# lucasnewman/f5-tts-mlx

Hardware: NVIDIA H100
Metric: mel-frames/sec (higher is better)
Workload: dtype bf16

## Files before the change

### f5_tts_mlx_b200/csrc/gemm_epilogue.cuh

```cuda
#pragma once
#include "ptx.cuh"

namespace f5 {

enum GemmAct { ACT_NONE = 0, ACT_GELU_TANH = 1, ACT_GELU_ERF = 2, ACT_MISH = 3 };

struct GemmParams {
  int M, N, K;
  int rows_per_batch;
  int tiles_per_batch;
  int num_batches;
  int conv_taps;
  int conv_pad;
  int k_per_tap;
  int conv_grouped;
  const float* bias;
  void* out;
  int ldo;
  const float* resid;
  int ldr;
  const float* gate;
  const int* row_len;
  const float2* rope;
  int rope_cols;
  int rope_col2;
  float q_scale;
  int q_cols;
  __nv_bfloat16* out2;
  int ldo2;
  unsigned long long* prof;
  int w_static;
  const char* pf_ptr;
  long long pf_bytes;
  const float* ln_scale;
  float2* ln_stats;
  const float2* ln_in_stats;
  int ln_in_units;
  const float* ln_tab;
  long long ln_tab_ld;
  int ab8;
  float acc_scale;
  int out2_fp8;
  int out_fp8;
  const float* a_scale;
  long long a_scale_ld;
  const float* w_scale;
  float* out_scale;
  float* out2_scale;
  int conv_dilation;
};

__device__ __forceinline__ void prefetch_slice_l2(const GemmParams& p, int cta, int num_ctas, int lane) {
  if (p.pf_ptr == nullptr) return;
  const long long per = (((p.pf_bytes + num_ctas - 1) / num_ctas) + 127) & ~127LL;
  const long long lo = (long long)cta * per;
  const long long hi = lo + per < p.pf_bytes ? lo + per : p.pf_bytes;
  for (long long o = lo + (long long)lane * 128; o < hi; o += 32 * 128)
    asm volatile("prefetch.global.L2 [%0];" ::"l"(p.pf_ptr + o));
}

__device__ __forceinline__ float tanh_approx(float x) {
  float y;
  asm("tanh.approx.f32 %0, %1;" : "=f"(y) : "f"(x));
  return y;
}
__device__ __forceinline__ float gelu_tanh_fast(float x) {
  const float k0 = 0.7978845608028654f, k1 = 0.044715f;
  const float u = k0 * fmaf(k1 * x * x, x, x);
  return 0.5f * x * (1.f + tanh_approx(u));
}
__device__ __forceinline__ float mish_fast(float x) {
  const float sp = x > 15.f ? x : __logf(1.f + __expf(x));
  return x * tanh_approx(sp);
}

template <int BN, bool SC = false>
__device__ __forceinline__ void epi_stage_cols(const GemmParams& p, int n0, int et, float* bias_s,
                                               float* gate_s, float* aux_s, float* ws_s = nullptr) {
#pragma unroll
  for (int i = et; i < BN; i += 128) {
    const int col = n0 + i;
    const bool ok = col < p.N;
    if constexpr (SC) ws_s[i] = (p.w_scale != nullptr && ok) ? p.acc_scale * p.w_scale[col] : p.acc_scale;
    float b = (p.bias != nullptr && ok) ? p.bias[col] : 0.f;
    float x = (p.ln_scale != nullptr && ok) ? 1.f + p.ln_scale[col] : 1.f;
    if (p.ln_in_stats != nullptr && ok) {
      const float* t = p.ln_tab + col;
      x = t[0] + t[p.ln_tab_ld];
      b += t[2 * p.ln_tab_ld] + t[3 * p.ln_tab_ld];
    }
    bias_s[i] = b;
    gate_s[i] = (p.gate != nullptr && ok) ? p.gate[col] : 1.f;
    aux_s[i] = x;
  }
}

__device__ __forceinline__ void epi_load_ln_row(const GemmParams& p, int row, bool row_ok, float& mu_r, float& rstd) {
  mu_r = 0.f; rstd = 1.f;
  if (p.ln_in_stats == nullptr || !row_ok) return;
  const float4* st = reinterpret_cast<const float4*>(p.ln_in_stats + (size_t)row * p.ln_in_units);
  float s1 = 0.f, s2 = 0.f;
  for (int u = 0; u < p.ln_in_units; u += 2) {
    const float4 v = st[u >> 1];
    s1 += v.x; s2 += v.y;
    s1 += v.z; s2 += v.w;
  }
  const float inv_k = 1.f / (64.f * p.ln_in_units);
  const float mean = s1 * inv_k;
  rstd = rsqrtf(fmaxf(s2 * inv_k - mean * mean, 0.f) + 1e-6f);
  mu_r = mean * rstd;
}

template <bool ROPE>
__device__ __forceinline__ void epi_load_rope(const GemmParams& p, int pos, float2 (&cs)[ROPE ? 32 : 1]) {
  if (ROPE) {
    const float4* rp = reinterpret_cast<const float4*>(p.rope + (size_t)pos * 32);
#pragma unroll
    for (int j = 0; j < 16; ++j) {
      const float4 v = rp[j];
      cs[2 * j] = make_float2(v.x, v.y);
      cs[2 * j + 1] = make_float2(v.z, v.w);
    }
  }
}

__device__ __forceinline__ void epi_load_resid(const GemmParams& p, int row, int col0, bool row_ok,
                                               float4 (&r)[8]) {
  if (p.resid != nullptr && row_ok && col0 < p.N) {
    const float4* rr = reinterpret_cast<const float4*>(p.resid + (size_t)row * p.ldr + col0);
#pragma unroll
    for (int j = 0; j < 8; ++j) r[j] = (col0 + 4 * j < p.N) ? rr[j] : make_float4(0.f, 0.f, 0.f, 0.f);
  } else {
#pragma unroll
    for (int j = 0; j < 8; ++j) r[j] = make_float4(0.f, 0.f, 0.f, 0.f);
  }
}

struct EpiStage {
  uint8_t* acc;
  uint8_t* stg;
  int et;
  int r;
  int bar_id;
  const CUtensorMap* map_out;
  const CUtensorMap* map_out2;
  int c1, c2;
  int out_fp8;
  float mu_r, rstd;
};

__device__ __forceinline__ void epi_stage_f32(uint8_t* buf, int r, const float (&v)[32]) {
  uint8_t* mine = buf + r * 128;
  const int sw = r & 7;
#pragma unroll
  for (int j = 0; j < 8; ++j)
    *reinterpret_cast<float4*>(mine + ((j ^ sw) * 16)) = make_float4(v[4 * j], v[4 * j + 1], v[4 * j + 2], v[4 * j + 3]);
}

template <bool OUT_BF16>
__device__ __forceinline__ void epi_store_tma(const float (&v)[32], const EpiStage& st, int ch, int col0,
                                              const uint4* w2 = nullptr, bool w2_fp8 = false) {
  uint8_t* box = st.acc + ch * 16384;
  uint8_t* buf = st.stg + (ch & 1) * 8192;
  if (OUT_BF16 && st.out_fp8) {
    uint8_t* mine = buf + st.r * 32;
    const int sw = (st.r >> 2) & 1;
#pragma unroll
    for (int j = 0; j < 2; ++j)
      *reinterpret_cast<uint4*>(mine + ((j ^ sw) * 16)) =
          make_uint4(pack_e4m3x4(v[16 * j], v[16 * j + 1], v[16 * j + 2], v[16 * j + 3]),
                     pack_e4m3x4(v[16 * j + 4], v[16 * j + 5], v[16 * j + 6], v[16 * j + 7]),
                     pack_e4m3x4(v[16 * j + 8], v[16 * j + 9], v[16 * j + 10], v[16 * j + 11]),
                     pack_e4m3x4(v[16 * j + 12], v[16 * j + 13], v[16 * j + 14], v[16 * j + 15]));
  } else if (OUT_BF16) {
    uint8_t* mine = buf + st.r * 64;
    const int sw = (st.r >> 1) & 3;
#pragma unroll
    for (int j = 0; j < 4; ++j)
      *reinterpret_cast<uint4*>(mine + ((j ^ sw) * 16)) =
          make_uint4(pack_bf16x2(v[8 * j], v[8 * j + 1]), pack_bf16x2(v[8 * j + 2], v[8 * j + 3]),
                     pack_bf16x2(v[8 * j + 4], v[8 * j + 5]), pack_bf16x2(v[8 * j + 6], v[8 * j + 7]));
  } else {
    epi_stage_f32(box, st.r, v);
  }
  if (w2 != nullptr) {
    if (w2_fp8) {
      uint8_t* mine2 = buf + st.r * 32;
      const int sw2 = (st.r >> 2) & 1;
#pragma unroll
      for (int j = 0; j < 2; ++j) *reinterpret_cast<uint4*>(mine2 + ((j ^ sw2) * 16)) = w2[j];
    } else {
      uint8_t* mine2 = buf + st.r * 64;
      const int sw2 = (st.r >> 1) & 3;
#pragma unroll
      for (int j = 0; j < 4; ++j) *reinterpret_cast<uint4*>(mine2 + ((j ^ sw2) * 16)) = w2[j];
    }
  }
  fence_proxy_async_smem();
  if (st.et == 0) tma_store_wait_read<0>();
  asm volatile("bar.sync %0, 128;" ::"r"(st.bar_id) : "memory");
  if (st.et == 0) {
    tma_store_3d(st.map_out, OUT_BF16 ? buf : box, col0, st.c1, st.c2);
    if (w2 != nullptr) tma_store_3d(st.map_out2, buf, col0, st.c1, st.c2);
    tma_store_commit();
  }
}


__device__ __forceinline__ void epi_quant32(const float (&v)[32], const float* aux, float inv, uint4 (&q)[2]) {
  uint32_t w[8];
#pragma unroll
  for (int i = 0; i < 8; ++i) {
    float x[4];
#pragma unroll
    for (int k = 0; k < 4; ++k) x[k] = (aux != nullptr ? v[4 * i + k] * aux[4 * i + k] : v[4 * i + k]) * inv;
    w[i] = pack_e4m3x4(x[0], x[1], x[2], x[3]);
  }
  q[0] = make_uint4(w[0], w[1], w[2], w[3]);
  q[1] = make_uint4(w[4], w[5], w[6], w[7]);
}

__device__ __forceinline__ void epi_quant32_staged(const uint8_t* buf, int r, const float* aux, float inv, uint4 (&q)[2]) {
  const uint8_t* mine = buf + r * 128;
  const int sw = r & 7;
  uint32_t w[8];
#pragma unroll
  for (int i = 0; i < 8; ++i) {
    const float4 a = *reinterpret_cast<const float4*>(mine + ((i ^ sw) * 16));
    float x[4] = {a.x, a.y, a.z, a.w};
#pragma unroll
    for (int k = 0; k < 4; ++k) x[k] = (aux != nullptr ? x[k] * aux[4 * i + k] : x[k]) * inv;
    w[i] = pack_e4m3x4(x[0], x[1], x[2], x[3]);
  }
  q[0] = make_uint4(w[0], w[1], w[2], w[3]);
  q[1] = make_uint4(w[4], w[5], w[6], w[7]);
}

template <bool OUT_BF16>
__device__ __forceinline__ void epi_finish_unit8(const float (&v)[32], const float* aux, float amax, float* scale,
                                                 int M, int colA, int row, bool row_ok, const EpiStage& st, int chA) {
  float inv;
  const float s = e4m3_block_scale(amax, inv);
  if (row_ok) scale[(size_t)(colA >> 6) * M + row] = s;
  uint8_t* q8 = st.stg + ((chA >> 1) & 1) * 8192;
  const int sw = (st.r >> 2) & 1;
  {
    uint4 q[2];
    epi_quant32(v, aux, inv, q);
#pragma unroll
    for (int j = 0; j < 2; ++j) *reinterpret_cast<uint4*>(q8 + 4096 + st.r * 32 + ((j ^ sw) * 16)) = q[j];
  }
  uint8_t* box_b = st.acc + (chA + 1) * 16384;
  if constexpr (!OUT_BF16) epi_stage_f32(box_b, st.r, v);
  {
    uint4 q[2];
    epi_quant32_staged(st.acc + chA * 16384, st.r, aux != nullptr ? aux - 32 : nullptr, inv, q);
#pragma unroll
    for (int j = 0; j < 2; ++j) *reinterpret_cast<uint4*>(q8 + st.r * 32 + ((j ^ sw) * 16)) = q[j];
  }
  fence_proxy_async_smem();
  if (st.et == 0) tma_store_wait_read<0>();
  asm volatile("bar.sync %0, 128;" ::"r"(st.bar_id) : "memory");
  if (st.et == 0) {
    if constexpr (!OUT_BF16) tma_store_3d(st.map_out, box_b, colA + 32, st.c1, st.c2);
    const CUtensorMap* m8 = OUT_BF16 ? st.map_out : st.map_out2;
    tma_store_3d(m8, q8, colA, st.c1, st.c2);
    tma_store_3d(m8, q8 + 4096, colA + 32, st.c1, st.c2);
    tma_store_commit();
  }
}

template <int ACT, bool OUT_BF16, bool ROPE, int HALF, bool SC = false>
__device__ __forceinline__ void epi_apply(const uint32_t (&acc)[32], const float4 (&res)[8],
                                          const float* bias_s, const float* gate_s, const float* aux_s,
                                          const float2 (&cs)[ROPE ? 32 : 1], const GemmParams& p,
                                          int col0, int ch, int row, bool row_ok, bool row_valid,
                                          const EpiStage& st, float2& unit_acc, const float* ws_s = nullptr,
                                          float* unit_amax = nullptr) {
  float v[32];
  if constexpr (SC) {
#pragma unroll
    for (int j = 0; j < 32; j += 4) {
      const float4 bb = *reinterpret_cast<const float4*>(bias_s + j);
      const float4 cc = *reinterpret_cast<const float4*>(aux_s + j);
      const float4 ww = *reinterpret_cast<const float4*>(ws_s + j);
      v[j] = fmaf(__uint_as_float(acc[j]), st.rstd * ww.x, fmaf(-st.mu_r, cc.x, bb.x));
      v[j + 1] = fmaf(__uint_as_float(acc[j + 1]), st.rstd * ww.y, fmaf(-st.mu_r, cc.y, bb.y));
      v[j + 2] = fmaf(__uint_as_float(acc[j + 2]), st.rstd * ww.z, fmaf(-st.mu_r, cc.z, bb.z));
      v[j + 3] = fmaf(__uint_as_float(acc[j + 3]), st.rstd * ww.w, fmaf(-st.mu_r, cc.w, bb.w));
    }
  } else if (p.ln_in_stats != nullptr) {
    const float ra = st.rstd * p.acc_scale;
#pragma unroll
    for (int j = 0; j < 32; j += 4) {
      const float4 bb = *reinterpret_cast<const float4*>(bias_s + j);
      const float4 cc = *reinterpret_cast<const float4*>(aux_s + j);
      v[j] = fmaf(__uint_as_float(acc[j]), ra, fmaf(-st.mu_r, cc.x, bb.x));
      v[j + 1] = fmaf(__uint_as_float(acc[j + 1]), ra, fmaf(-st.mu_r, cc.y, bb.y));
      v[j + 2] = fmaf(__uint_as_float(acc[j + 2]), ra, fmaf(-st.mu_r, cc.z, bb.z));
      v[j + 3] = fmaf(__uint_as_float(acc[j + 3]), ra, fmaf(-st.mu_r, cc.w, bb.w));
    }
  } else {
#pragma unroll
    for (int j = 0; j < 32; j += 4) {
      const float4 bb = *reinterpret_cast<const float4*>(bias_s + j);
      v[j] = fmaf(__uint_as_float(acc[j]), p.acc_scale, bb.x);
      v[j + 1] = fmaf(__uint_as_float(acc[j + 1]), p.acc_scale, bb.y);
      v[j + 2] = fmaf(__uint_as_float(acc[j + 2]), p.acc_scale, bb.z);
      v[j + 3] = fmaf(__uint_as_float(acc[j + 3]), p.acc_scale, bb.w);
    }
  }
  if (ACT == ACT_GELU_TANH) {
#pragma unroll
    for (int j = 0; j < 32; ++j) v[j] = gelu_tanh_fast(v[j]);
  } else if (ACT == ACT_GELU_ERF) {
#pragma unroll
    for (int j = 0; j < 32; ++j) v[j] = gelu_erf_f(v[j]);
  } else if (ACT == ACT_MISH) {
#pragma unroll
    for (int j = 0; j < 32; ++j) v[j] = mish_fast(v[j]);
  }
  if (ROPE) {
    if (col0 < p.rope_cols || (unsigned)(col0 - p.rope_col2) < (unsigned)p.rope_cols) {
#pragma unroll
      for (int j = 0; j < 16; ++j) {
        const float2 c = cs[HALF * 16 + j];
        const float a = v[2 * j], b = v[2 * j + 1];
        v[2 * j] = a * c.x - b * c.y;
        v[2 * j + 1] = b * c.x + a * c.y;
      }
    }
    if (col0 < p.q_cols) {
#pragma unroll
      for (int j = 0; j < 32; ++j) v[j] *= p.q_scale;
    }
  }
  if (p.row_len != nullptr) {
    if (!row_valid) {
#pragma unroll
      for (int j = 0; j < 32; ++j) v[j] = 0.f;
    }
  }
#pragma unroll
  for (int j = 0; j < 8; ++j) {
    const float4 gg = *reinterpret_cast<const float4*>(gate_s + 4 * j);
    v[4 * j] = fmaf(v[4 * j], gg.x, res[j].x); v[4 * j + 1] = fmaf(v[4 * j + 1], gg.y, res[j].y);
    v[4 * j + 2] = fmaf(v[4 * j + 2], gg.z, res[j].z); v[4 * j + 3] = fmaf(v[4 * j + 3], gg.w, res[j].w);
  }
  if constexpr (!OUT_BF16) {
    if (p.out2 != nullptr) {
      if (p.ln_stats != nullptr) {
        float s1[4] = {HALF == 0 ? 0.f : unit_acc.x, 0.f, 0.f, 0.f}, s2[4] = {HALF == 0 ? 0.f : unit_acc.y, 0.f, 0.f, 0.f};
#pragma unroll
        for (int j = 0; j < 32; j += 4) {
#pragma unroll
          for (int i = 0; i < 4; ++i) { s1[i] += v[j + i]; s2[i] = fmaf(v[j + i], v[j + i], s2[i]); }
        }
        unit_acc = make_float2((s1[0] + s1[1]) + (s1[2] + s1[3]), (s2[0] + s2[1]) + (s2[2] + s2[3]));
        if (HALF == 1 && row_ok && col0 < p.N) p.ln_stats[(size_t)row * (p.N >> 6) + (col0 >> 6)] = unit_acc;
      }
      if constexpr (SC) {
        if (p.out2_fp8 && p.out2_scale != nullptr) {
          float amax = HALF == 0 ? 0.f : *unit_amax;
#pragma unroll
          for (int j = 0; j < 32; ++j) amax = fmax_nan(amax, fabsf(v[j] * aux_s[j]));
          if (HALF == 0) {
            *unit_amax = amax;
            epi_store_tma<OUT_BF16>(v, st, ch, col0);
          } else {
            epi_finish_unit8<OUT_BF16>(v, aux_s, amax, p.out2_scale, p.M, col0 - 32, row, row_ok, st, ch - 1);
          }
          return;
        }
      }
      uint4 w2[4];
      if (p.out2_fp8) {
#pragma unroll
        for (int j = 0; j < 2; ++j) {
          uint32_t q[4];
#pragma unroll
          for (int i = 0; i < 4; ++i) {
            const float4 sc = *reinterpret_cast<const float4*>(aux_s + 16 * j + 4 * i);
            q[i] = pack_e4m3x4(v[16 * j + 4 * i] * sc.x, v[16 * j + 4 * i + 1] * sc.y, v[16 * j + 4 * i + 2] * sc.z,
                               v[16 * j + 4 * i + 3] * sc.w);
          }
          w2[j] = make_uint4(q[0], q[1], q[2], q[3]);
        }
      } else {
#pragma unroll
        for (int j = 0; j < 4; ++j) {
          const float4 s0 = *reinterpret_cast<const float4*>(aux_s + 8 * j);
          const float4 s1 = *reinterpret_cast<const float4*>(aux_s + 8 * j + 4);
          w2[j] = make_uint4(pack_bf16x2(v[8 * j] * s0.x, v[8 * j + 1] * s0.y), pack_bf16x2(v[8 * j + 2] * s0.z, v[8 * j + 3] * s0.w),
                             pack_bf16x2(v[8 * j + 4] * s1.x, v[8 * j + 5] * s1.y), pack_bf16x2(v[8 * j + 6] * s1.z, v[8 * j + 7] * s1.w));
        }
      }
      epi_store_tma<OUT_BF16>(v, st, ch, col0, w2, p.out2_fp8 != 0);
      return;
    }
  }
  if constexpr (SC && OUT_BF16) {
    if (st.out_fp8 && p.out_scale != nullptr) {
      float amax = HALF == 0 ? 0.f : *unit_amax;
#pragma unroll
      for (int j = 0; j < 32; ++j) amax = fmax_nan(amax, fabsf(v[j]));
      if (HALF == 0) {
        *unit_amax = amax;
        epi_stage_f32(st.acc + ch * 16384, st.r, v);
      } else {
        epi_finish_unit8<OUT_BF16>(v, nullptr, amax, p.out_scale, p.M, col0 - 32, row, row_ok, st, ch - 1);
      }
      return;
    }
  }
  epi_store_tma<OUT_BF16>(v, st, ch, col0);
}

__device__ __forceinline__ void acc_ld32(const uint8_t* box, int r, uint32_t (&acc)[32]) {
  const uint8_t* mine = box + r * 128;
  const int sw = r & 7;
#pragma unroll
  for (int j = 0; j < 8; ++j) {
    const float4 v = *reinterpret_cast<const float4*>(mine + ((j ^ sw) * 16));
    acc[4 * j] = __float_as_uint(v.x); acc[4 * j + 1] = __float_as_uint(v.y);
    acc[4 * j + 2] = __float_as_uint(v.z); acc[4 * j + 3] = __float_as_uint(v.w);
  }
}

template <int BN, int ACT, bool OUT_BF16, bool ROPE, bool SC = false>
__device__ __forceinline__ void epi_drain_tile(const float* bias_s, const float* gate_s, const float* aux_s,
                                               const float2 (&cs)[ROPE ? 32 : 1], float4 (&res0)[8], const GemmParams& p,
                                               int n0, int row, bool row_ok, bool row_valid, const EpiStage& st,
                                               const float* ws_s = nullptr) {
  float4 res1[8];
  float2 unit_acc = make_float2(0.f, 0.f);
  float unit_amax = 0.f;
#pragma unroll 1
  for (int cc = 0; cc < BN / 64; ++cc) {
    const int colA = n0 + cc * 64, colB = colA + 32;
    uint32_t acc[32];
    constexpr bool kLateB = ROPE || SC;
    if (kLateB || cc > 0) epi_load_resid(p, row, colA, row_ok, res0);
    if constexpr (!kLateB) epi_load_resid(p, row, colB, row_ok, res1);
    acc_ld32(st.acc + (2 * cc) * 16384, st.r, acc);
    if (colA < p.N)
      epi_apply<ACT, OUT_BF16, ROPE, 0, SC>(acc, res0, bias_s + cc * 64, gate_s + cc * 64, aux_s + cc * 64, cs, p, colA,
                                            2 * cc, row, row_ok, row_valid, st, unit_acc, SC ? ws_s + cc * 64 : nullptr,
                                            &unit_amax);
    if constexpr (kLateB) epi_load_resid(p, row, colB, row_ok, res1);
    acc_ld32(st.acc + (2 * cc + 1) * 16384, st.r, acc);
    if (colB < p.N)
      epi_apply<ACT, OUT_BF16, ROPE, 1, SC>(acc, res1, bias_s + cc * 64 + 32, gate_s + cc * 64 + 32, aux_s + cc * 64 + 32, cs,
                                            p, colB, 2 * cc + 1, row, row_ok, row_valid, st, unit_acc,
                                            SC ? ws_s + cc * 64 + 32 : nullptr, &unit_amax);
  }
}

}
```

### f5_tts_mlx_b200/csrc/gemm_sm90.cuh

```cuda
#pragma once
#include <type_traits>

#include "ptx.cuh"
#include "gemm_epilogue.cuh"

namespace f5 {

template <int BN, int kStages, bool SCALED = false>
struct GemmSmem {
  static constexpr int kABytes = 128 * 128;
  static constexpr int kBBytes = BN * 128;
  static constexpr int kStageBytes = kABytes + kBBytes;
  static constexpr int kAccOffset = kStages * kStageBytes;
  static constexpr int kAccBytes = (BN / 32) * 16384;
  static constexpr int kStgOffset = kAccOffset + kAccBytes;
  static constexpr int kBarOffset = kStgOffset + 16384;
  static constexpr int kColsOffset = (kBarOffset + (2 * kStages + 2) * 8 + 15) & ~15;
  static constexpr int kTotal = kColsOffset + (SCALED ? 4 : 3) * BN * 4 + 1024;
  static_assert(kStageBytes % 1024 == 0, "SWIZZLE_128B tiles and boxes sit on 1024-byte boundaries");
  static_assert(kTotal <= 232448, "GEMM: shared memory over the 227 KB limit");
};

template <int BN>
struct GemmEpi {
  static constexpr int kThreads = 384;
};

template <int BN, bool AB8>
__device__ __forceinline__ void gemm_wgmma(float (&acc)[BN / 2], uint64_t da, uint64_t db, uint32_t scale_d) {
  if constexpr (AB8) {
    if constexpr (BN == 128) wgmma_e4m3_ss_n128(acc, da, db, scale_d);
    else wgmma_e4m3_ss_n64(acc, da, db, scale_d);
  } else {
    if constexpr (BN == 128) wgmma_bf16_ss_n128(acc, da, db, scale_d);
    else wgmma_bf16_ss_n64(acc, da, db, scale_d);
  }
}

struct GemmTile {
  int n0;
  int batch;
  int m_in_batch0;
  int row0;
};
__device__ __forceinline__ GemmTile gemm_tile(const GemmParams& p, int t, int bn) {
  GemmTile g;
  const int tiles_n = (p.N + bn - 1) / bn;
  const int mt = t / tiles_n;
  g.n0 = (t - mt * tiles_n) * bn;
  if (p.tiles_per_batch > 0) {
    g.batch = mt / p.tiles_per_batch;
    g.m_in_batch0 = (mt - g.batch * p.tiles_per_batch) * 128;
    g.row0 = g.batch * p.rows_per_batch + g.m_in_batch0;
  } else {
    g.batch = 0;
    g.row0 = mt * 128;
    g.m_in_batch0 = g.row0;
  }
  return g;
}
__device__ __forceinline__ int gemm_tiles(const GemmParams& p, int bn) {
  return (p.N + bn - 1) / bn * (p.tiles_per_batch > 0 ? p.num_batches * p.tiles_per_batch : (p.M + 127) / 128);
}
__device__ __forceinline__ int gemm_num_kb(const GemmParams& p) {
  return p.conv_taps * (p.ab8 ? (p.k_per_tap + 127) >> 7 : (p.k_per_tap + 63) >> 6);
}

template <int BN, int kStages, int ACT, bool OUT_BF16, bool ROPE, bool FP8 = false, bool RESID = true, bool SCALED = false>
__global__ void __launch_bounds__(384, 1)
gemm_bf16_tn_kernel(const __grid_constant__ CUtensorMap tma_a,
                    const __grid_constant__ CUtensorMap tma_b, const __grid_constant__ CUtensorMap tma_out,
                    const __grid_constant__ CUtensorMap tma_out2, const GemmParams p_arg) {
  GemmParams p = p_arg;
  if constexpr (!FP8) { p.ab8 = 0; p.out_fp8 = 0; p.out2_fp8 = 0; p.acc_scale = 1.f; }
  if constexpr (!RESID) p.resid = nullptr;
  if constexpr (!SCALED) { p.a_scale = nullptr; p.w_scale = nullptr; p.out_scale = nullptr; p.out2_scale = nullptr; }
  using S = GemmSmem<BN, kStages, SCALED>;
  extern __shared__ uint8_t smem_raw[];
  uint8_t* smem = smem_raw + ((1024u - (smem_u32(smem_raw) & 1023u)) & 1023u);
  uint64_t* full_bar = reinterpret_cast<uint64_t*>(smem + S::kBarOffset);
  uint64_t* empty_bar = full_bar + kStages;
  uint64_t* mma_turn = empty_bar + kStages;
  uint64_t* epi_free = mma_turn + 1;

  const int warp = threadIdx.x >> 5;
  const int lane = threadIdx.x & 31;

  if (warp == 0 && elect_one()) {
    tma_prefetch_desc(&tma_a);
    tma_prefetch_desc(&tma_b);
    tma_prefetch_desc(&tma_out);
    if (p.out2 != nullptr) tma_prefetch_desc(&tma_out2);
    for (int i = 0; i < kStages; ++i) {
      mbar_init(&full_bar[i], 1);
      mbar_init(&empty_bar[i], 128);
    }
    mbar_init(mma_turn, 128);
    mbar_init(epi_free, 128);
    fence_mbar_init();
  }
  if (warp == 1) prefetch_slice_l2(p, blockIdx.x, gridDim.x, lane);
  __syncthreads();
  const int early_b = p.w_static ? min(kStages, gemm_num_kb(p)) : 0;
  if (warp == 0 && elect_one()) {
    const int n0 = gemm_tile(p, blockIdx.x, BN).n0;
    for (int kb = 0; kb < early_b; ++kb) {
      mbar_expect_tx(&full_bar[kb], S::kStageBytes);
      tma_load_2d(smem + kb * S::kStageBytes + S::kABytes, &tma_b, &full_bar[kb], kb * (p.ab8 ? 128 : 64), n0);
    }
  }
  pdl_wait();
  if (threadIdx.x == 128) prof_stamp_begin(p.prof);

  if (warp < 4) {
    asm volatile("setmaxnreg.dec.sync.aligned.u32 40;\n");
    if (warp == 0 && elect_one()) {
      auto produce = [&](auto ab8_tag) {
        constexpr int KBE = decltype(ab8_tag)::value ? 128 : 64;
        const int kb_per_tap = (p.k_per_tap + KBE - 1) / KBE, num_kb = p.conv_taps * kb_per_tap, tiles = gemm_tiles(p, BN);
        const int tap_step = p.conv_dilation > 1 ? p.conv_dilation : 1;
        int s = 0;
        uint32_t ph = 1;
        uint8_t* sa = smem;
        int early = p.w_static ? min(kStages, num_kb) : 0;
        for (int t = blockIdx.x; t < tiles; t += gridDim.x) {
          const GemmTile g = gemm_tile(p, t, BN);
          const int a_col0 = p.conv_grouped ? g.n0 : 0;
          int a_row = g.m_in_batch0 - p.conv_pad, kc = 0;
          for (int kb = 0; kb < num_kb; ++kb) {
            mbar_wait(&empty_bar[s], ph);
            if (kb >= early) mbar_expect_tx(&full_bar[s], S::kStageBytes);
            tma_load_3d(sa, &tma_a, &full_bar[s], a_col0 + kc * KBE, a_row, g.batch);
            if (kb >= early) tma_load_2d(sa + S::kABytes, &tma_b, &full_bar[s], kb * KBE, g.n0);
            if (++s == kStages) { s = 0; ph ^= 1; sa = smem; } else { sa += S::kStageBytes; }
            if (++kc == kb_per_tap) { kc = 0; a_row += tap_step; }
          }
          early = 0;
        }
      };
      if (p.ab8) produce(std::true_type{});
      else produce(std::false_type{});
    }
  } else {
    asm volatile("setmaxnreg.inc.sync.aligned.u32 232;\n");
    const int wg = (threadIdx.x >> 7) - 1;
    const int et = threadIdx.x & 127;
    const int wr = ((threadIdx.x >> 5) & 3) * 16 + (lane >> 2);
    const uint32_t ring = smem_u32(smem);
    uint8_t* acc_tile = smem + S::kAccOffset;
    float* bias_s = reinterpret_cast<float*>(smem + S::kColsOffset);
    float* gate_s = bias_s + BN;
    float* aux_s = bias_s + 2 * BN;
    float* ws_s = SCALED ? bias_s + 3 * BN : nullptr;

    const uint32_t turn_par = (uint32_t)wg ^ 1u;
#pragma unroll 1
    for (int t = blockIdx.x + wg * gridDim.x; t < gemm_tiles(p, BN); t += 2 * gridDim.x) {
      const int num_kb = gemm_num_kb(p);
      const bool first = t == (int)blockIdx.x;
      const int kb0 = (t - (int)blockIdx.x) / (int)gridDim.x * num_kb;
      int s = kb0 % kStages;
      uint32_t ph = (uint32_t)(kb0 / kStages) & 1u;
      if (!first) mbar_wait(mma_turn, turn_par);

      float acc[2][BN / 2];
#pragma unroll
      for (int h = 0; h < 2; ++h)
#pragma unroll
        for (int i = 0; i < BN / 2; ++i) acc[h][i] = 0.f;
      auto mma_loop = [&](auto ab8_tag) {
        constexpr bool AB8 = decltype(ab8_tag)::value;
        if constexpr (AB8) {
          float part[BN / 2];
          for (int kb = 0; kb < num_kb; ++kb) {
            mbar_wait(&full_bar[s], ph);
            const uint32_t sa = ring + s * S::kStageBytes, sb = ring + s * S::kStageBytes + S::kABytes;
#pragma unroll
            for (int h = 0; h < 2; ++h) {
              wgmma_fence();
#pragma unroll
              for (int k = 0; k < 4; ++k)
                gemm_wgmma<BN, true>(part, gmma_desc_sw128(sa + h * (64 * 128) + 32 * k, 16, 1024),
                                     gmma_desc_sw128(sb + 32 * k, 16, 1024), k != 0);
              wgmma_commit();
              wgmma_wait<0>();
              wgmma_reg_fence(part);
              if (h == 1) mbar_arrive(&empty_bar[s]);
#pragma unroll
              for (int i = 0; i < BN / 2; ++i) acc[h][i] += part[i];
            }
            if (++s == kStages) { s = 0; ph ^= 1; }
          }
        } else {
          int s_prev = 0;
          for (int kb = 0; kb < num_kb; ++kb) {
            mbar_wait(&full_bar[s], ph);
            const uint32_t sa = ring + s * S::kStageBytes, sb = ring + s * S::kStageBytes + S::kABytes;
            wgmma_fence();
#pragma unroll
            for (int h = 0; h < 2; ++h)
#pragma unroll
              for (int k = 0; k < 4; ++k)
                gemm_wgmma<BN, false>(acc[h], gmma_desc_sw128(sa + h * (64 * 128) + 32 * k, 16, 1024),
                                      gmma_desc_sw128(sb + 32 * k, 16, 1024), (kb | k) != 0);
            wgmma_commit();
            wgmma_wait<1>();
            if (kb > 0) mbar_arrive(&empty_bar[s_prev]);
            s_prev = s;
            if (++s == kStages) { s = 0; ph ^= 1; }
          }
          wgmma_wait<0>();
          wgmma_reg_fence(acc[0]);
          wgmma_reg_fence(acc[1]);
          mbar_arrive(&empty_bar[s_prev]);
        }
      };
      auto mma_loop_scaled = [&]() {
        const GemmTile g = gemm_tile(p, t, BN);
        const int lim = p.tiles_per_batch > 0 ? p.rows_per_batch - g.m_in_batch0 : p.M - g.row0;
        const float* sp = p.a_scale + g.row0 + wr;
        const size_t ld = (size_t)p.a_scale_ld;
        float part[BN / 2];
        for (int kb = 0; kb < num_kb; ++kb) {
          float sc[2][2][2];
#pragma unroll
          for (int u = 0; u < 2; ++u) {
            const float* su = sp + (size_t)(2 * kb + u) * ld;
#pragma unroll
            for (int h = 0; h < 2; ++h) {
              sc[u][h][0] = 64 * h + wr < lim ? su[64 * h] : 0.f;
              sc[u][h][1] = 64 * h + wr + 8 < lim ? su[64 * h + 8] : 0.f;
            }
          }
          mbar_wait(&full_bar[s], ph);
          const uint32_t sa = ring + s * S::kStageBytes, sb = ring + s * S::kStageBytes + S::kABytes;
#pragma unroll
          for (int u = 0; u < 2; ++u) {
#pragma unroll
            for (int h = 0; h < 2; ++h) {
              wgmma_fence();
#pragma unroll
              for (int k = 0; k < 2; ++k)
                gemm_wgmma<BN, true>(part, gmma_desc_sw128(sa + h * (64 * 128) + 64 * u + 32 * k, 16, 1024),
                                     gmma_desc_sw128(sb + 64 * u + 32 * k, 16, 1024), k != 0);
              wgmma_commit();
              wgmma_wait<0>();
              wgmma_reg_fence(part);
              if (u == 1 && h == 1) mbar_arrive(&empty_bar[s]);
#pragma unroll
              for (int i = 0; i < BN / 2; ++i) acc[h][i] = fmaf(part[i], sc[u][h][(i >> 1) & 1], acc[h][i]);
            }
          }
          if (++s == kStages) { s = 0; ph ^= 1; }
        }
      };
      if constexpr (SCALED) {
        if (p.ab8 && p.a_scale != nullptr) mma_loop_scaled();
        else if (p.ab8) mma_loop(std::true_type{});
        else mma_loop(std::false_type{});
      } else {
        if (p.ab8) mma_loop(std::true_type{});
        else mma_loop(std::false_type{});
      }
      mbar_arrive(mma_turn);
      if (t + (int)gridDim.x >= gemm_tiles(p, BN)) pdl_launch_dependents();

      const GemmTile g = gemm_tile(p, t, BN);
      if (!first) mbar_wait(epi_free, turn_par);
      {
        const int sw = wr & 7;
        uint8_t* base = acc_tile + wr * 128 + (lane & 1) * 8;
#pragma unroll
        for (int h = 0; h < 2; ++h)
#pragma unroll
          for (int q = 0; q < BN / 8; ++q) {
            uint8_t* pc = base + h * (64 * 128) + (q >> 2) * 16384 + (((2 * (q & 3) + ((lane >> 1) & 1)) ^ sw) << 4);
            *reinterpret_cast<float2*>(pc) = make_float2(acc[h][4 * q], acc[h][4 * q + 1]);
            *reinterpret_cast<float2*>(pc + 8 * 128) = make_float2(acc[h][4 * q + 2], acc[h][4 * q + 3]);
          }
      }
      epi_stage_cols<BN, SCALED>(p, g.n0, et, bias_s, gate_s, aux_s, ws_s);
      const int m_in_batch = g.m_in_batch0 + et;
      const int row = g.row0 + et;
      bool row_ok;
      int b_idx, pos;
      if (p.tiles_per_batch > 0) {
        row_ok = m_in_batch < p.rows_per_batch;
        b_idx = g.batch;
        pos = m_in_batch;
      } else {
        row_ok = row < p.M;
        const int rpb = p.rows_per_batch > 0 ? p.rows_per_batch : p.M;
        b_idx = row / rpb;
        pos = row - b_idx * rpb;
      }
      if (!row_ok) { b_idx = 0; pos = 0; }
      bool row_valid = true;
      if (p.row_len != nullptr) row_valid = pos < p.row_len[b_idx];
      float ln_mu_r, ln_rstd;
      epi_load_ln_row(p, row, row_ok, ln_mu_r, ln_rstd);
      float2 cs[ROPE ? 32 : 1];
      epi_load_rope<ROPE>(p, pos, cs);
      float4 res0[8];
      if constexpr (!(ROPE || SCALED)) epi_load_resid(p, row, g.n0, row_ok, res0);
      EpiStage stg;
      stg.acc = acc_tile;
      stg.stg = smem + S::kStgOffset;
      stg.et = et;
      stg.r = et;
      stg.map_out = &tma_out;
      stg.map_out2 = &tma_out2;
      stg.c1 = g.m_in_batch0;
      stg.c2 = g.batch;
      stg.bar_id = 1 + wg;
      stg.mu_r = ln_mu_r; stg.rstd = ln_rstd;
      stg.out_fp8 = p.out_fp8;
      asm volatile("bar.sync %0, 128;" ::"r"(stg.bar_id) : "memory");
      epi_drain_tile<BN, ACT, OUT_BF16, ROPE, SCALED>(bias_s, gate_s, aux_s, cs, res0, p, g.n0, row, row_ok, row_valid,
                                                      stg, ws_s);
      if (et == 0) tma_store_wait_read<0>();
      mbar_arrive(epi_free);
    }
  }

  __syncthreads();
  if (threadIdx.x == 0) prof_stamp_end(p.prof);
}

}
```

Baseline: 10770.

## Split last-tile epilogue across both consumer warpgroups to cut tail latency

For BN=128 non-scaled GEMMs, the idle consumer warpgroup now takes the second 64-column half of the other warpgroup's final tile epilogue. The tile-loop bound gets one extra iteration that does no MMA, only epilogue. The two warpgroups meet at a shared 256-thread named barrier and use the stage ring memory as the helper's staging buffer. This is meant to shorten the serialized tail epilogue per CTA, at the cost of extra synchronization and reuse of pipeline smem that could race with TMA loads.

```diff
diff --git a/f5_tts_mlx_b200/csrc/gemm_epilogue.cuh b/f5_tts_mlx_b200/csrc/gemm_epilogue.cuh
--- a/f5_tts_mlx_b200/csrc/gemm_epilogue.cuh
+++ b/f5_tts_mlx_b200/csrc/gemm_epilogue.cuh
@@ -431,12 +431,12 @@
 __device__ __forceinline__ void epi_drain_tile(const float* bias_s, const float* gate_s, const float* aux_s,
                                                const float2 (&cs)[ROPE ? 32 : 1], float4 (&res0)[8], const GemmParams& p,
                                                int n0, int row, bool row_ok, bool row_valid, const EpiStage& st,
-                                               const float* ws_s = nullptr) {
+                                               const float* ws_s, int units) {
   float4 res1[8];
   float2 unit_acc = make_float2(0.f, 0.f);
   float unit_amax = 0.f;
 #pragma unroll 1
-  for (int cc = 0; cc < BN / 64; ++cc) {
+  for (int cc = 0; cc < units; ++cc) {
     const int colA = n0 + cc * 64, colB = colA + 32;
     uint32_t acc[32];
     constexpr bool kLateB = ROPE || SC;
diff --git a/f5_tts_mlx_b200/csrc/gemm_sm90.cuh b/f5_tts_mlx_b200/csrc/gemm_sm90.cuh
--- a/f5_tts_mlx_b200/csrc/gemm_sm90.cuh
+++ b/f5_tts_mlx_b200/csrc/gemm_sm90.cuh
@@ -154,8 +154,13 @@
     float* ws_s = SCALED ? bias_s + 3 * BN : nullptr;
 
     const uint32_t turn_par = (uint32_t)wg ^ 1u;
+    constexpr bool kSplitLast = BN == 128 && !SCALED && !(FP8 && ROPE);
 #pragma unroll 1
-    for (int t = blockIdx.x + wg * gridDim.x; t < gemm_tiles(p, BN); t += 2 * gridDim.x) {
+    for (int t = blockIdx.x + wg * gridDim.x; t < gemm_tiles(p, BN) + (kSplitLast ? (int)gridDim.x : 0);
+         t += 2 * gridDim.x) {
+      const bool help = kSplitLast && t >= gemm_tiles(p, BN);
+      GemmTile g;
+      if (!help) {
       const int num_kb = gemm_num_kb(p);
       const bool first = t == (int)blockIdx.x;
       const int kb0 = (t - (int)blockIdx.x) / (int)gridDim.x * num_kb;
@@ -265,7 +270,7 @@
       mbar_arrive(mma_turn);
       if (t + (int)gridDim.x >= gemm_tiles(p, BN)) pdl_launch_dependents();
 
-      const GemmTile g = gemm_tile(p, t, BN);
+      g = gemm_tile(p, t, BN);
       if (!first) mbar_wait(epi_free, turn_par);
       {
         const int sw = wr & 7;
@@ -280,6 +285,11 @@
           }
       }
       epi_stage_cols<BN, SCALED>(p, g.n0, et, bias_s, gate_s, aux_s, ws_s);
+      }
+
+      if (help) g = gemm_tile(p, t - (int)gridDim.x, BN);
+      const int c0 = help ? 64 : 0;
+      const int units = kSplitLast && (help || t + (int)gridDim.x >= gemm_tiles(p, BN)) ? 1 : BN / 64;
       const int m_in_batch = g.m_in_batch0 + et;
       const int row = g.row0 + et;
       bool row_ok;
@@ -302,10 +312,10 @@
       float2 cs[ROPE ? 32 : 1];
       epi_load_rope<ROPE>(p, pos, cs);
       float4 res0[8];
-      if constexpr (!(ROPE || SCALED)) epi_load_resid(p, row, g.n0, row_ok, res0);
+      if constexpr (!(ROPE || SCALED)) epi_load_resid(p, row, g.n0 + c0, row_ok, res0);
       EpiStage stg;
-      stg.acc = acc_tile;
-      stg.stg = smem + S::kStgOffset;
+      stg.acc = acc_tile + c0 * 512;
+      stg.stg = c0 != 0 ? smem : smem + S::kStgOffset;
       stg.et = et;
       stg.r = et;
       stg.map_out = &tma_out;
@@ -315,10 +325,13 @@
       stg.bar_id = 1 + wg;
       stg.mu_r = ln_mu_r; stg.rstd = ln_rstd;
       stg.out_fp8 = p.out_fp8;
-      asm volatile("bar.sync %0, 128;" ::"r"(stg.bar_id) : "memory");
-      epi_drain_tile<BN, ACT, OUT_BF16, ROPE, SCALED>(bias_s, gate_s, aux_s, cs, res0, p, g.n0, row, row_ok, row_valid,
-                                                      stg, ws_s);
+      if (kSplitLast && units == 1) asm volatile("bar.sync 3, 256;" ::: "memory");
+      else asm volatile("bar.sync %0, 128;" ::"r"(stg.bar_id) : "memory");
+      epi_drain_tile<BN, ACT, OUT_BF16, ROPE, SCALED>(bias_s + c0, gate_s + c0, aux_s + c0, cs, res0, p, g.n0 + c0, row,
+                                                      row_ok, row_valid, stg, SCALED ? ws_s + c0 : nullptr,
+                                                      units);
       if (et == 0) tma_store_wait_read<0>();
+      if (c0 != 0) break;
       mbar_arrive(epi_free);
     }
   }
```

Result: faster. 11000, median of 6 (+2.2%).
